# kylc/optik

Hardware: AMD Instinct MI355X
Metric: random-restart IK solves/sec (Panda 7-DoF, 1e-6 tol) (higher is better)
Workload: dtype f64

## Files before the change

include/optik_hip.h:

```cpp
#ifndef OPTIK_HIP_H
#define OPTIK_HIP_H

#include <stdint.h>

#ifdef __cplusplus
extern "C" {
#endif

#define OPTIK_HIP_MAX_DOF 16

enum {
    OPTIK_HIP_OK = 0,
    OPTIK_HIP_EINVAL = -1,
    OPTIK_HIP_EUNSUPPORTED = -2,
    OPTIK_HIP_ENODEVICE = -3,
    OPTIK_HIP_ENOMEM = -4
};

enum { OPTIK_JOINT_FIXED = 0, OPTIK_JOINT_REVOLUTE = 1, OPTIK_JOINT_PRISMATIC = 2 };

enum {
    OPTIK_RES_FAILURE = -1,
    OPTIK_RES_ROUNDOFF_LIMITED = -4,
    OPTIK_RES_FORCED_STOP = -5,
// ... 46 lines not shown
int optik_hip_diff_ik_batch(const optik_hip_chain *chain, const double *ee_offset7, const double *d_q,
                            const double *d_V, int64_t ld_V, const double *d_vmax, int64_t ld_vmax,
                            int64_t B, double *d_alpha, double *d_v, int32_t *d_status, void *stream);

int optik_hip_manip_batch(const optik_hip_chain *chain, const double *ee_offset7, const double *d_q, int64_t B,
                          double *d_w, double *d_c, void *stream);

#define OPTIK_HIP_MAX_COLLISION_SPHERES 256
#define OPTIK_HIP_MAX_COLLISION_PAIRS 4096
#define OPTIK_HIP_MAX_WORLD_OBSTACLES 65536
int optik_hip_chain_set_collision_model(optik_hip_chain *chain, const int32_t *frames, const double *centers3,
                                        const double *radii, int32_t S, const int32_t *pairs2, int32_t P,
                                        double margin);
int optik_hip_chain_set_world(optik_hip_chain *chain, const double *spheres4, int32_t Ms, const double *boxes10,
                              int32_t Mb);
int optik_hip_link_frames_batch(const optik_hip_chain *chain, const double *ee_offset7, const double *d_q, int64_t B,
                                double *d_frames, void *stream);
int optik_hip_collision_batch(const optik_hip_chain *chain, const double *ee_offset7, const double *d_q, int64_t B,
                              double *d_clearance, uint8_t *d_free, void *stream);

int optik_hip_seed_batch(const optik_hip_chain *chain, uint64_t first, int64_t count, double *d_q,
                         void *stream);

#define OPTIK_HIP_IK_EARLY_EXIT 1u
#define OPTIK_HIP_IK_FIND_ANY 2u
#define OPTIK_HIP_IK_RESTART_MAJOR 4u
typedef struct optik_hip_ik_outputs {
    double *d_x;
    double *d_f;
    int32_t *d_status;
    int32_t *d_evals;
    double *d_win_x;
    double *d_win_f;
    uint64_t *d_win_idx;
    double *d_win_key;
} optik_hip_ik_outputs;

int optik_hip_ik_batch(optik_hip_chain *chain, const optik_solver_config *cfg,
                       const double *d_targets, const double *d_x0, int32_t T,
                       const double *ee_offset7, uint64_t restart_begin, uint64_t restart_end,
                       uint32_t flags, double deadline_s, const optik_hip_ik_outputs *out,
                       void *stream);

#define OPTIK_HIP_MAX_SOLUTIONS 256
typedef struct optik_hip_ik_solutions_outputs {
    int32_t *d_count;
// ... 50 lines not shown
```

optik_amd/_native.py:

```python
from __future__ import annotations

import ctypes as C
import os

_HERE = os.path.dirname(os.path.abspath(__file__))
LIB_PATH = os.path.join(_HERE, "csrc", "liboptik_amd.so")
if os.environ.get("OPTIK_AMD_LIB"):
    LIB_PATH = os.path.abspath(os.environ["OPTIK_AMD_LIB"])

MAX_DOF = 8
IK_EARLY_EXIT = 1
IK_FIND_ANY = 2
IK_RESTART_MAJOR = 4
UINT64_MAX = 0xFFFFFFFFFFFFFFFF

RES_FAILURE, RES_ROUNDOFF, RES_FORCED_STOP, RES_ITER_CAP = -1, -4, -5, -100
RES_STOPVAL, RES_FTOL, RES_XTOL = 2, 3, 4
RANGE_SINGLE_INCLUSIVE, RANGE_NEW_INCLUSIVE = 0, 1


class OptikHipError(RuntimeError):
    pass


# ... 63 lines not shown
def lib():
    global _lib
    if _lib is not None:
        return _lib
    if not os.path.exists(LIB_PATH):
        raise OptikHipError(
            f"{LIB_PATH} is missing: build it with `python -c 'import __graft_entry__ as g; "
            "g.build()'` (hipcc --offload-arch=gfx950).  optik_amd has no CPU fallback.")
    L = C.CDLL(LIB_PATH, mode=C.RTLD_GLOBAL)
    vp, dp, ip = C.c_void_p, C.POINTER(C.c_double), C.POINTER(C.c_int32)
    L.optik_hip_device_count.restype = C.c_int
    L.optik_hip_set_option.argtypes = [C.c_char_p, C.c_longlong]
    L.optik_hip_get_option.argtypes = [C.c_char_p]
    L.optik_hip_get_option.restype = C.c_longlong
    L.optik_hip_last_error.restype = C.c_char_p
    L.optik_hip_chain_create.argtypes = [dp, dp, ip, C.c_int32, dp, dp, C.c_int32, C.POINTER(vp)]
    L.optik_hip_chain_destroy.argtypes = [vp]
    L.optik_hip_chain_num_positions.argtypes = [vp]
    L.optik_hip_chain_set_range_rule.argtypes = [vp, C.c_int32]
    L.optik_hip_chain_range_rule.argtypes = [vp]
    L.optik_hip_eval_batch.argtypes = [vp, C.POINTER(SolverConfigC), dp, dp, vp, C.c_int64, vp, vp, vp]
    L.optik_hip_fk_batch.argtypes = [vp, dp, vp, C.c_int64, vp, vp, vp]
    L.optik_hip_seed_batch.argtypes = [vp, C.c_uint64, C.c_int64, vp, vp]
    L.optik_hip_manip_batch.argtypes = [vp, dp, vp, C.c_int64, vp, vp, vp]
    ip = C.POINTER(C.c_int32)
    L.optik_hip_chain_set_collision_model.argtypes = [vp, ip, dp, dp, C.c_int32, ip, C.c_int32, C.c_double]
    L.optik_hip_chain_set_world.argtypes = [vp, dp, C.c_int32, dp, C.c_int32]
    L.optik_hip_link_frames_batch.argtypes = [vp, dp, vp, C.c_int64, vp, vp]
    L.optik_hip_collision_batch.argtypes = [vp, dp, vp, C.c_int64, vp, vp, vp]
    L.optik_hip_diff_ik_batch.argtypes = [vp, dp, vp, vp, C.c_int64, vp, C.c_int64, C.c_int64, vp, vp, vp, vp]
    L.optik_hip_ik_batch.argtypes = [vp, C.POINTER(SolverConfigC), vp, vp, C.c_int32, dp,
                                     C.c_uint64, C.c_uint64, C.c_uint32, C.c_double,
                                     C.POINTER(IkOutputs), vp]
    L.optik_hip_ik_solutions.argtypes = [vp, C.POINTER(SolverConfigC), vp, vp, C.c_int32, dp, C.c_uint64,
                                         C.c_uint64, C.c_double, C.c_int32, C.c_double,
                                         C.POINTER(IkSolutionsOutputs), vp]
    L.optik_hip_ik_path.argtypes = [vp, C.POINTER(SolverConfigC), vp, vp, C.c_int32, C.c_int32, dp, C.c_uint64,
                                    C.c_uint64, C.c_uint32, C.c_double, C.c_double, C.POINTER(IkPathOutputs), vp]
    L.optik_hip_ik_host.argtypes = [vp, C.POINTER(SolverConfigC), dp, dp, C.c_int32, dp,
                                    C.c_uint64, C.c_uint64, C.c_uint32, C.c_double, dp, dp,
                                    C.POINTER(C.c_uint64), dp]
    L.optik_hip_probe.argtypes = [C.c_int32, dp, dp, C.c_int64, dp]
    L.optik_hip_probe_math.argtypes = [C.c_int32, dp, C.c_int64, dp]
    L.optik_hip_set_timing.argtypes = [vp, C.c_int32]
    L.optik_hip_last_launch.argtypes = [vp, C.POINTER(LaunchInfo)]
    L.optik_hip_timing_mean.argtypes = [vp, C.POINTER(C.c_double), C.POINTER(C.c_int32)]
# ... 63 lines not shown
```

optik_amd/csrc/ik_batch_ops.hip:

```cpp
#include "diff_ik_lp.hpp"
#include "ik_host.hpp"
#include "ik_jacobian.hpp"

using namespace optik;
using namespace optik::host;
using namespace optik::hostparams;

namespace {

struct EvalLaunch {
    const ChainDev *chain;
    EvalParams ep;
    double target[7];
    const double *q;
    long long B;
    double *f;
    double *g;
};

template <int N, bool TIP>
__global__ __launch_bounds__(256) void eval_batch_kernel(const EvalLaunch a) {
    __shared__ ChainDev sch;
    stage_chain(sch, a.chain);
    const Pose target = load_pose(a.target);
// ... 140 lines not shown
        const double p[7] = {ee.t.x, ee.t.y, ee.t.z, ee.q.i, ee.q.j, ee.q.k, ee.q.w};
#pragma unroll
        for (int i = 0; i < 7; ++i) a.pose[(size_t)i * a.B + b] = p[i];
    }
}

struct SeedLaunch {
    uint32_t key[8];
    double lb[MAX_DOF];
    double scale[MAX_DOF];
    unsigned long long first;
    long long count;
    double *q;
};

template <int N>
__global__ __launch_bounds__(256) void seed_batch_kernel(const SeedLaunch a) {
    for (long long b = (long long)blockIdx.x * blockDim.x + threadIdx.x; b < a.count;
         b += (long long)gridDim.x * blockDim.x) {
        double q[N];
        restart_seed<N>(a.key, a.lb, a.scale, a.first + (unsigned long long)b, q);
#pragma unroll
        for (int i = 0; i < N; ++i) a.q[(size_t)i * a.count + b] = q[i];
    }
}

__global__ void probe_kernel(int op, const double *a, const double *b, long long count, double *out) {
    for (long long i = (long long)blockIdx.x * blockDim.x + threadIdx.x; i < count;
         i += (long long)gridDim.x * blockDim.x) {
        double r = 0.0, s, c;
        switch (op) {
        case 0: r = a[i] / b[i]; break;
        case 1: r = __builtin_sqrt(a[i]); break;
        case 2: sincos_dev(a[i], s, c); r = s; break;
        case 3: sincos_dev(a[i], s, c); r = c; break;
        default: r = atan2_q1(a[i], b[i]); break;
        }
        out[i] = r;
    }
}

__global__ void probe_math_kernel(int op, const double *poses, long long count, double *out, int stride) {
    for (long long i = (long long)blockIdx.x * blockDim.x + threadIdx.x; i < count;
         i += (long long)gridDim.x * blockDim.x) {
        const Pose X = load_pose(poses + i * 7);
        double *o = out + i * stride;
// ... 4 lines not shown
        if (op == 1) {
            for (int r = 0; r < 3; ++r) for (int c = 0; c < 3; ++c) o[r * 3 + c] = Jr.m[r][c];
        } else if (op == 2) {
            const V3 lin = se3_log_linear(rt, X.t);
            o[0] = lin.x; o[1] = lin.y; o[2] = lin.z; o[3] = w.x; o[4] = w.y; o[5] = w.z;
        } else {
            const M3 Q = se3_q_matrix(rt, X.t, Jr);
            for (int r = 0; r < 3; ++r)
                for (int c = 0; c < 3; ++c) {
                    o[r * 6 + c] = Jr.m[r][c];
                    o[r * 6 + 3 + c] = Q.m[r][c];
                    o[(r + 3) * 6 + c] = 0.0;
                    o[(r + 3) * 6 + 3 + c] = Jr.m[r][c];
                }
        }
    }
}

const char *const kPrismaticJacobianMsg =
    "joint_jacobian: prismatic joints are not implemented (the reference panics: kinematics.rs:185 todo!())";

}

extern "C" {

int optik_hip_eval_batch(const optik_hip_chain *ch, const optik_solver_config *cfg, const double *target7,
                         const double *ee_offset7, const double *d_q, int64_t B, double *d_f, double *d_g,
                         void *stream) {
    if (!ch || !cfg || !target7 || !d_q || !d_f || B < 0) return fail(OPTIK_HIP_EINVAL, "bad argument");
    if (B == 0) return 0;
    if (ch->prismatic)
        return fail(OPTIK_HIP_EUNSUPPORTED,
                    "prismatic joints: only forward kinematics is available (the reference's Jacobian panics, kinematics.rs:185)");
    BIND_DEVICE(ch);
    if (ch->wide) {
        WideBatchLaunch w;
        std::memset(&w, 0, sizeof w);
        w.chain = ch->wdev;
        make_eval_params(cfg->linear_weight, cfg->angular_weight, ee_offset7, w.ep);
        std::memcpy(w.target, target7, sizeof w.target);
        w.q = d_q; w.B = B; w.f = d_f; w.g = d_g;
        HIP_TRY(wide_batch_launch(0, grid_for(ch, B, 256, 8), (hipStream_t)stream, w));
        return 0;
    }
    EvalLaunch a;
    a.chain = ch->dev;
// ... 87 lines not shown
    BIND_DEVICE(ch);
    if (ch->wide) {
        WideBatchLaunch w;
        std::memset(&w, 0, sizeof w);
        w.chain = ch->wdev;
        std::memcpy(w.key, ch->key, sizeof w.key);
        w.first = first; w.B = count; w.q_out = d_q;
        HIP_TRY(wide_batch_launch(2, grid_for(ch, count, 256, 8), (hipStream_t)stream, w));
        return 0;
    }
    SeedLaunch a;
    std::memcpy(a.key, ch->key, sizeof a.key);
    std::memcpy(a.lb, ch->host.lb, sizeof a.lb);
    std::memcpy(a.scale, ch->scale, sizeof a.scale);
    a.first = first; a.count = count; a.q = d_q;
    const int grid = grid_for(ch, count, 256, 8);
#define CALL(NN, TT) hipLaunchKernelGGL((seed_batch_kernel<NN>), dim3(grid), dim3(256), 0, (hipStream_t)stream, a)
    OPTIK_DISPATCH(ch, CALL);
#undef CALL
    HIP_TRY(hipGetLastError());
    return 0;
}

int optik_hip_probe(int32_t op, const double *a, const double *b, int64_t count, double *out) {
    if (!a || !out || count < 0) return fail(OPTIK_HIP_EINVAL, "bad argument");
    if (int rc = ensure_device()) return rc;
    if (count == 0) return 0;
    double *d_a = nullptr, *d_b = nullptr, *d_o = nullptr;
    const size_t bytes = sizeof(double) * (size_t)count;
    HIP_TRY(hipMalloc(&d_a, bytes));
    HIP_TRY(hipMalloc(&d_b, bytes));
    HIP_TRY(hipMalloc(&d_o, bytes));
    HIP_TRY(hipMemcpy(d_a, a, bytes, hipMemcpyHostToDevice));
    HIP_TRY(hipMemcpy(d_b, b ? b : a, bytes, hipMemcpyHostToDevice));
    hipLaunchKernelGGL(probe_kernel, dim3(1024), dim3(256), 0, nullptr, op, d_a, d_b, (long long)count, d_o);
    HIP_TRY(hipGetLastError());
    HIP_TRY(hipMemcpy(out, d_o, bytes, hipMemcpyDeviceToHost));
    hipFree(d_a); hipFree(d_b); hipFree(d_o);
    return 0;
}

int optik_hip_probe_math(int32_t op, const double *poses7, int64_t count, double *out) {
    if (!poses7 || !out || count < 0 || op < 0 || op > 3) return fail(OPTIK_HIP_EINVAL, "bad argument");
    if (int rc = ensure_device()) return rc;
    if (count == 0) return 0;
    const int stride = op == 0 ? 3 : (op == 1 ? 9 : (op == 2 ? 6 : 36));
// ... 15 lines not shown
```

optik_amd/csrc/ik_capi.hip:

```cpp
#include <algorithm>
#include <cstdio>
#include <cstdlib>
#include <vector>

#include "ik_host.hpp"

using namespace optik;
using namespace optik::host;
using namespace optik::hostparams;

namespace optik {
namespace host {

thread_local std::string g_err;

static int solve_kernel_from(const char *e) {
    if (!e) return SK_AUTO;
    if (!std::strcmp(e, "quad")) return SK_QUAD;
    if (!std::strcmp(e, "lane64")) return SK_LANE64;
    if (!std::strcmp(e, "general")) return SK_GENERAL;
    return SK_AUTO;
}
Options &opt() {
    static Options o = [] {
        Options v;
        v.solve_kernel = solve_kernel_from(std::getenv("OPTIK_SOLVE_KERNEL"));
        if (const char *e = std::getenv("OPTIK_WIDE_FORM")) v.wide_form = std::strcmp(e, "hbm") == 0 ? 1 : 0;
        if (const char *e = std::getenv("OPTIK_RANDOM_RANGE_RULE"))
            if (std::strcmp(e, "new_inclusive") == 0 || std::strcmp(e, "1") == 0) v.range_rule = OPTIK_HIP_RANGE_NEW_INCLUSIVE;
        return v;
    }();
    return o;
}

}
}

namespace {

int default_range_rule() { return opt().range_rule; }

void set_chain_scales(optik_hip_chain *ch, int rule) {
    ch->range_rule = rule;
    for (int k = 0; k < ch->n; ++k) {
        const double lb = ch->wide ? ch->whost.lb[k] : ch->host.lb[k], ub = ch->wide ? ch->whost.ub[k] : ch->host.ub[k];
        ch->scale[k] = (std::isfinite(lb) && std::isfinite(ub)) ? uniform_scale(lb, ub, rule) : NAN;
        if (ch->wide) ch->whost.scale[k] = ch->scale[k];
    }
}

}

// ... 91 lines not shown
    hipDeviceGetAttribute(&ch->wall_clock_khz, hipDeviceAttributeWallClockRate, dev);
    *out = ch;
    return 0;
}

void optik_hip_chain_destroy(optik_hip_chain *ch) {
    if (!ch) return;
    optik::DeviceScope dev_scope(ch->device_id);
    if (ch->claim_pending) (void)hipStreamSynchronize(nullptr);
    if (ch->dev) hipFree(ch->dev);
    if (ch->wdev) hipFree(ch->wdev);
    if (ch->wide_ws) hipFree(ch->wide_ws);
    if (ch->tile_recs) hipFree(ch->tile_recs);
    if (ch->first_success) hipFree(ch->first_success);
    if (ch->sol_pick) hipFree(ch->sol_pick);
    if (ch->path_carry) hipFree(ch->path_carry);
    if (ch->coll_dev) hipFree(ch->coll_dev);
    if (ch->world_dev) hipFree(ch->world_dev);
    if (ch->tmp_x) hipFree(ch->tmp_x);
    if (ch->tmp_f) hipFree(ch->tmp_f);
    if (ch->tmp_key) hipFree(ch->tmp_key);
    if (ch->queue) hipFree(ch->queue);
    if (ch->hw_dev) hipFree(ch->hw_dev);
    if (ch->hw_pin) hipHostFree(ch->hw_pin);
    if (ch->hw_claim) hipHostFree(ch->hw_claim);
    if (ch->claim_done) hipEventDestroy(ch->claim_done);
    for (int i = 0; i < optik_hip_chain::EV_POOL; ++i) {
        if (ch->ev0[i]) hipEventDestroy(ch->ev0[i]);
        if (ch->ev1[i]) hipEventDestroy(ch->ev1[i]);
    }
    delete ch;
}

int32_t optik_hip_chain_num_positions(const optik_hip_chain *ch) { return ch ? ch->n : 0; }

int optik_hip_chain_set_range_rule(optik_hip_chain *ch, int32_t rule) {
    if (!ch || (rule != OPTIK_HIP_RANGE_SINGLE_INCLUSIVE && rule != OPTIK_HIP_RANGE_NEW_INCLUSIVE))
        return fail(OPTIK_HIP_EINVAL, "bad argument");
    std::lock_guard<std::mutex> lock(ch->mu);
    set_chain_scales(ch, rule);
    if (ch->wide) {
        BIND_DEVICE(ch);
        HIP_TRY(hipMemcpy(ch->wdev, &ch->whost, sizeof(WideChainDev), hipMemcpyHostToDevice));
    }
    return 0;
}

int32_t optik_hip_chain_range_rule(const optik_hip_chain *ch) { return ch ? ch->range_rule : -1; }

}

struct SolvedLaunch {
    double *px, *pf, *pk;
    uint64_t R;
    uint64_t tiles_per_target;
    size_t cols;
    size_t fs_clean_after;
    bool early;
};

static int solve_locked(optik_hip_chain *ch, const optik_solver_config *cfg, const double *d_targets,
                        const double *d_x0, int32_t T, const double *ee_offset7, uint64_t restart_begin,
                        uint64_t restart_end, uint32_t flags, double deadline_s, const optik_hip_ik_outputs *out,
// ... 204 lines not shown
    if (early && (flags & OPTIK_HIP_IK_RESTART_MAJOR) && resident > (long long)T * inflight) {
        const long long floor_res = std::max(2 * cap, (long long)T * 32);
        resident = std::max((long long)T * inflight, std::min(resident, floor_res));
    }
    long long lanes = (resident + cap - 1) / cap;
    if (lanes < 1) lanes = 1;
    if (lanes > per_wave_max) lanes = per_wave_max;
    bool wide_lds = false;
    if (widek) {
        wide_lds = opt().wide_form != 1;
        if (wide_lds) lanes = 1;
    }
    a.wq.lanes = (int)lanes;
    if (claim_request && quadk && !lanek && a.wq.find_any && T == 1 && ch->hw_claim) {
        a.wq.claim = ch->hw_claim;
        a.wq.claim_seq = ++ch->claim_seq;
        if (claim_armed) *claim_armed = true;
        if (stream == nullptr) ch->claim_pending = true;
    }
    long long grid_ll = (resident + lanes - 1) / lanes;
    if (grid_ll > cap) grid_ll = cap;
    const int grid = (int)grid_ll;

    const int ev_slot = ch->ev_count % optik_hip_chain::EV_POOL;
    if (ch->timing) {
        if (!ch->ev0[ev_slot]) { HIP_TRY(hipEventCreate(&ch->ev0[ev_slot])); HIP_TRY(hipEventCreate(&ch->ev1[ev_slot])); }
        HIP_TRY(hipEventRecord(ch->ev0[ev_slot], stream));
    }
    int lds = 0;
    if (widek) {
        const bool lds_form = wide_lds;
        if (!lds_form && (size_t)grid > ch->wide_ws_waves) {
            if (ch->wide_ws) HIP_TRY(hipFree(ch->wide_ws));
            ch->wide_ws = nullptr; ch->wide_ws_waves = 0;
            HIP_TRY(hipMalloc(&ch->wide_ws, sizeof(double) * wide_ws_doubles_per_wave() * (size_t)grid));
            ch->wide_ws_waves = (size_t)grid;
        }
        WideSolveLaunch w;
        std::memset(&w, 0, sizeof w);
        w.chain = ch->wdev;
        w.ep = a.ep; w.sp = a.sp; w.wq = a.wq;
        std::memcpy(w.key, ch->key, sizeof w.key);
        w.deadline_ticks = a.deadline_ticks;
        w.ws = ch->wide_ws;
        lds = lds_form ? wide_lds_bytes() : (int)sizeof(WideChainDev);
        HIP_TRY(wide_solve_launch(grid, stream, w, lds_form, opt().wide_form != 2));
// ... 120 lines not shown
        s.x = out->d_x ? out->d_x + w * (size_t)n : nullptr;
        s.f = out->d_f ? out->d_f + w : nullptr;
        s.idx = out->d_idx ? (unsigned long long *)out->d_idx + w : nullptr;
        s.key = out->d_key ? out->d_key + w : nullptr;
        s.step = out->d_step ? out->d_step + w : nullptr;
        s.reset_queue = ch->queue;
        s.reset_fs = sl.early ? ch->first_success : nullptr;
        HIP_TRY(path_select_launch(s, P, stream));
        ch->queue_clean = true;
        ch->fs_clean = sl.fs_clean_after;
        ch->clean_stream = stream;
    }
    return 0;
}

static long long *option_slot(const char *name, int **islot) {
    Options &o = opt();
    *islot = nullptr;
    if (!name) return nullptr;
    if (!std::strcmp(name, "solve_kernel")) { *islot = &o.solve_kernel; return nullptr; }
    if (!std::strcmp(name, "wide_form")) { *islot = &o.wide_form; return nullptr; }
    if (!std::strcmp(name, "range_rule")) { *islot = &o.range_rule; return nullptr; }
    if (!std::strcmp(name, "stop_x_legacy")) { *islot = &o.stop_x_legacy; return nullptr; }
    return nullptr;
}
int optik_hip_set_option(const char *name, long long value) {
    int *is = nullptr;
    long long *ls = option_slot(name, &is);
    if (ls) { *ls = value; return 0; }
    if (is) { *is = (int)value; return 0; }
    return fail(OPTIK_HIP_EINVAL, "unknown option");
}
long long optik_hip_get_option(const char *name) {
    int *is = nullptr;
    long long *ls = option_slot(name, &is);
    return ls ? *ls : (is ? (long long)*is : -1);
}

int optik_hip_ik_host(optik_hip_chain *ch, const optik_solver_config *cfg, const double *targets,
                      const double *x0, int32_t T, const double *ee_offset7, uint64_t restart_begin,
                      uint64_t restart_end, uint32_t flags, double deadline_s, double *win_x, double *win_f,
                      uint64_t *win_idx, double *win_key) {
    if (!ch || !cfg || !targets || !x0 || T < 1) return fail(OPTIK_HIP_EINVAL, "bad argument");
    std::lock_guard<std::mutex> host_lock(ch->host_mu);
    BIND_DEVICE(ch);
    const int n = ch->n;
// ... 132 lines not shown
```

optik_amd/csrc/ik_host.hpp:

```cpp
#pragma once

#include <hip/hip_runtime.h>

#include <cmath>
#include <cstring>
#include <mutex>
#include <string>

#include "../../include/optik_hip.h"
#include "device_scope.hpp"
#include "ik_host_params.hpp"
#include "ik_launch.hpp"
#include "ik_wide_launch.hpp"

namespace optik {
namespace coll {
struct ModelDev;
}
namespace host {

constexpr int WAVE = 64;
constexpr int QUADS_PER_WAVE_HOST = 16;

struct TileRec {
// ... 57 lines not shown
    int n;
    int filter;
    double max_step;
    unsigned long long restart_begin;
    unsigned long long n_restarts;
    size_t ld;
    double *x;
    double *f;
    unsigned long long *idx;
    double *key;
    double *step;
    unsigned long long *reset_queue;
    unsigned long long *reset_fs;
};
hipError_t path_select_launch(const PathSelectLaunch &s, int P, hipStream_t stream);

int manip_key_launch(const optik_hip_chain *ch, int mode, const double *ee_offset7, const double *x, double *key,
                     size_t cols, hipStream_t stream);

int collision_key_launch(const optik_hip_chain *ch, const double *ee_offset7, const double *x, double *key,
                         size_t cols, hipStream_t stream);

enum : int { SK_AUTO = 0, SK_QUAD = 1, SK_LANE64 = 2, SK_GENERAL = 3 };
struct Options {
    int solve_kernel = SK_AUTO;
    int wide_form = 0;
    int range_rule = OPTIK_HIP_RANGE_SINGLE_INCLUSIVE;
    int stop_x_legacy = 0;
};
Options &opt();

extern thread_local std::string g_err;
inline int fail(int code, const std::string &msg) {
    g_err = msg;
    return code;
}

#define HIP_TRY(expr)                                                                   \
    do {                                                                                \
        hipError_t e_ = (expr);                                                         \
        if (e_ != hipSuccess)                                                           \
            return ::optik::host::fail(OPTIK_HIP_ENODEVICE, std::string(#expr) + ": " + hipGetErrorString(e_)); \
    } while (0)

inline int ensure_device() {
    int n = 0;
    hipError_t e = hipGetDeviceCount(&n);
    if (e != hipSuccess || n <= 0)
        return fail(OPTIK_HIP_ENODEVICE, std::string("no HIP device available: ")
                                             + (e == hipSuccess ? "device count is 0" : hipGetErrorString(e)));
    return 0;
// ... 52 lines not shown
    size_t sol_pick_cap = 0;
    double *path_carry = nullptr;
    size_t path_carry_cap = 0;
    int coll_S = 0, coll_P = 0, coll_groups = 0;
    double coll_margin = 0.0;
    optik::coll::ModelDev *coll_dev = nullptr;
    double *world_dev = nullptr;
    size_t world_cap = 0;
    int world_Ms = 0, world_Mb = 0;
    bool queue_clean = false;
    size_t fs_clean = 0;
    hipStream_t clean_stream = nullptr;
    double *tmp_x = nullptr, *tmp_f = nullptr, *tmp_key = nullptr;
    size_t tmp_cols = 0;
    unsigned long long *queue = nullptr;
    unsigned long long *prof = nullptr;
    double *hw_dev = nullptr, *hw_pin = nullptr;
    size_t hw_cap = 0;
    unsigned long long *hw_claim = nullptr;
    hipEvent_t claim_done = nullptr;
    unsigned long long claim_seq = 0;
    bool claim_pending = false;
    unsigned hw_flip = 0;
    int timing = 0;
    static constexpr int EV_POOL = 256;
    hipEvent_t ev0[EV_POOL] = {}, ev1[EV_POOL] = {};
    int ev_count = 0;
    optik_hip_launch_info last{};
    int num_cus = 0;
    int wall_clock_khz = 0;
};

namespace optik {
namespace host {

inline int grid_for(const optik_hip_chain *ch, long long work, int block, int per_cu) {
    long long blocks = (work + block - 1) / block;
    const long long cap = (long long)(ch->num_cus > 0 ? ch->num_cus : 256) * per_cu;
    if (blocks > cap) blocks = cap;
    if (blocks < 1) blocks = 1;
    return (int)blocks;
}

}
}
```

optik_amd/csrc/ik_lane64.hpp:

```cpp
#pragma once

#include "ik_lane.hpp"
#include "ik_solve.hpp"
#include "ik_nnls_quad.hpp"

namespace optik {

template <int N>
struct Lane64Geom {
    static constexpr int NG = N * (N + 1) / 2;
    static constexpr int REC = NG + 2 * N;
    OPTIK_DEV static constexpr int g(int i, int j) { return i * N - (i * (i - 1)) / 2 + (j - i); }
    OPTIK_DEV static constexpr int hlo(int i) { return NG + i; }
    OPTIK_DEV static constexpr int hhi(int i) { return NG + N + i; }
    static constexpr int META = NnlsQuadGeom<N>::XS + 2 * N;
    static_assert(NnlsQuadGeom<N>::XS + 2 * N + 3 <= NnlsQuadGeom<N>::STRIDE, "three spare doubles per block");
};

}
#include "ik_nnls_first.hpp"
namespace optik {

#ifndef OPTIK_LANE_FIRST_PASS_MIN
#define OPTIK_LANE_FIRST_PASS_MIN 16
// ... 7 lines not shown

template <int N>
constexpr int lane64_block_lds() { return nnls_quad_wave_lds<N>(); }
template <int N>
constexpr int lane64_rec_lds() { return Lane64Geom<N>::REC * 64; }

#ifndef OPTIK_LANE_CLASSES
#define OPTIK_LANE_CLASSES 8
#endif
constexpr int LANE64_CLASSES = OPTIK_LANE_CLASSES;
#ifndef OPTIK_LANE_PIPE
#define OPTIK_LANE_PIPE 1
#endif
#ifndef LANE64_MAX_RUNNING
#define LANE64_MAX_RUNNING 14
#endif
#ifndef OPTIK_LANE_RESERVE
#define OPTIK_LANE_RESERVE 8
#endif
#ifndef OPTIK_LANE_KEEP_TARGET
#define OPTIK_LANE_KEEP_TARGET 1
#endif
#ifndef OPTIK_LANE_REFILL
#define OPTIK_LANE_REFILL 4
#endif

template <int N, class Expand, class ReadBack>
struct Lane64Pipe {
    static constexpr bool on = true;
    static constexpr bool warm_start = true;
    static constexpr int MAX_RUNNING = LANE64_MAX_RUNNING;
    int n_prob, next, hold;
    int qi, ql, lane, rank;
    bool has, got;
    double *bk;
    int *lor, *where;
    Expand *expand_fn;
    ReadBack *read_fn;
    OPTIK_DEV bool more() const { return next < n_prob; }
    template <bool WARM>
    OPTIK_DEV bool event(bool idle, int mode, double rn, int passes, double *wst, int &wj) {
        wj = 0;
        const bool fin = idle && hold >= 0;
        if (wave_any(fin)) {
            if (fin && ql == 0) {
                bk[Lane64Geom<N>::META] = (double)mode;
                bk[Lane64Geom<N>::META + 1] = rn;
                bk[Lane64Geom<N>::META + 2] = (double)passes;
// ... 8 lines not shown
            if (fin) hold = -1;
        }
        const bool free_q = idle && hold < 0;
        const unsigned long long fm = __ballot(free_q);
        const int mine = (int)__popcll(fm & ((1ull << (lane & ~3)) - 1ull)) / QUAD;
        const int pr = next + mine;
        const bool live = free_q && pr < n_prob;
        next += (int)__popcll(fm) / QUAD;
        next = next < n_prob ? next : n_prob;
        if (wave_any(live)) {
            const int p = lor[live ? pr : 0];
            (*expand_fn)(std::integral_constant<bool, WARM>{}, live, p, wst, wj);
            if (live) hold = pr;
        }
        return live;
    }
};

template <int N, bool TIP>
OPTIK_DEV void lane64_wave(const ChainDev &ch, const EvalParams &ep, const SolveParams &sp, const uint32_t (&key)[8],
                           const double (&scale)[MAX_DOF], const WorkQueue &wq,
                           double *nnls_lds ,
                           double *rec_lds , int *lor_lds ,
                           int *where_lds ) {
    typedef Lane64Geom<N> G;
    constexpr int NL = N * (N + 1) / 2;
    constexpr int NS = (N > 4) ? 2 : 1;
    constexpr int CS = NnlsQuadGeom<N>::CS;
    static_assert(N <= 7, "the throughput form of chains with at most seven joints");
    const double alfmin = 0.1;
    const int lane = (int)(threadIdx.x & 63u);
    double x[N], x0[N], g[N], s[N], l[NL];
    double xbest[N], xprev[N];
    double f = 0.0, f0 = 0.0, t0 = 0.0, h3 = 0.0, alpha = 1.0;
    double minf = __builtin_huge_val(), fprev = __builtin_huge_val();
    int ireset = 0, line = 0, nevals = 0;
    int pred = 1;
    bool first = true;
    bool again = false;
    Pose target;
    unsigned long long item = 0, index = 0;
    unsigned tslot = OPTIK_LANE_KEEP_TARGET ? ~0u : 0u;
    bool active = false, want = lane < wq.lanes;
#if OPTIK_LANE_RESERVE > 0
    unsigned long long rbase = 0, rend = 0;
    unsigned long long pend = 0;
    bool r_pending = false;
    bool dry = false;
#endif
#pragma unroll
    for (int i = 0; i < N; ++i) { x[i] = 0.0; x0[i] = 0.0; g[i] = 0.0; s[i] = 0.0; xbest[i] = 0.0; xprev[i] = 0.0; }
#pragma unroll
    for (int i = 0; i < NL; ++i) l[i] = 0.0;
    target.t = V3{0, 0, 0};
    target.q = Q4{0, 0, 0, 1};

#ifdef OPTIK_PROFILE
    unsigned long long lp_[8] = {0, 0, 0, 0, 0, 0, 0, 0};
    unsigned long long lt_ = __builtin_readcyclecounter();
#define LANE_PROF(slot) do { const unsigned long long n_ = __builtin_readcyclecounter(); lp_[slot] += n_ - lt_; lt_ = n_; } while (0)
#else
#define LANE_PROF(slot)
#endif
    for (;;) {
        const unsigned n_want = (unsigned)__popcll(__ballot(want));
        if (n_want >= (unsigned)(wq.lanes < OPTIK_LANE_REFILL ? wq.lanes : OPTIK_LANE_REFILL) || (n_want > 0 && !wave_any(active))) {
#if OPTIK_LANE_RESERVE > 0
            unsigned long long it;
            {
                if (r_pending) { rbase = __shfl(pend, 0); rend = rbase + OPTIK_LANE_RESERVE; r_pending = false; }
                const unsigned long long wm = __ballot(want);
                const unsigned rank = (unsigned)__popcll(wm & ((1ull << lane) - 1ull));
                const unsigned long long have = rend - rbase;
                const unsigned long long take = n_want < have ? n_want : have;
                it = rbase + rank;
                rbase += take;
                if (wave_any(want && rank >= take)) {
                    const unsigned long long it2 = fetch_items(wq.next_item, want && rank >= take);
                    if (rank >= take) it = it2;
                }
                dry = dry || wave_any(want && it >= wq.total_items);
            }
#else
            const unsigned long long it = fetch_items(wq.next_item, want);
#endif
            if (want) {
                want = false;
                if (it < wq.total_items) {
                    unsigned long long r;
#if OPTIK_LANE_KEEP_TARGET
                    const unsigned tprev = tslot;
#endif
                    if (wq.restart_major) { r = it / wq.n_targets; tslot = (unsigned)(it - r * wq.n_targets); }
                    else { tslot = (unsigned)(it / wq.n_restarts); r = it - (unsigned long long)tslot * wq.n_restarts; }
                    item = (unsigned long long)tslot * wq.n_restarts + r;
                    index = wq.restart_begin + r;
#if OPTIK_LANE_KEEP_TARGET
                    if (tslot != tprev) target = load_pose(wq.targets + (size_t)tslot * 7);
#else
                    target = load_pose(wq.targets + (size_t)tslot * 7);
#endif
                    restart_seed<N>(key, ch.lb, scale, index, x);
                    if (index == 0) {
                        const double *x0p = wq.x0 + (size_t)tslot * N;
#pragma unroll
                        for (int i = 0; i < N; ++i) x[i] = x0p[i];
                    }
#pragma unroll
                    for (int i = 0; i < N; ++i) { xbest[i] = x[i]; xprev[i] = x[i]; x0[i] = x[i]; s[i] = 0.0; g[i] = 0.0; }
                    f = 0.0; f0 = 0.0; t0 = 0.0; h3 = 0.0; alpha = 1.0;
                    minf = __builtin_huge_val(); fprev = __builtin_huge_val();
                    ireset = 0; line = 0; nevals = 0; pred = 1;
                    first = true;
                    again = false;
                    active = true;
                }
            }
        }
#if OPTIK_LANE_RESERVE > 0
        if (!r_pending && rbase == rend && !dry) {
            if (lane == 0) pend = atomicAdd(wq.next_item, (unsigned long long)OPTIK_LANE_RESERVE);
            r_pending = true;
        }
#endif
        if (!wave_any(active)) break;
        LANE_PROF(0);

        int32_t ret = 0;
        if (active) {
            bool stop = false;
            if (wq.first_success) {
                const unsigned long long fs = __hip_atomic_load(wq.first_success + tslot, __ATOMIC_RELAXED,
                                                                __HIP_MEMORY_SCOPE_AGENT);
                stop = wq.find_any ? (fs != ~0ull) : (fs < index);
            }
            if (wq.deadline && (unsigned long long)wall_clock64() > wq.deadline) stop = true;
            if (stop) ret = RES_FORCED_STOP;
        }
        const bool stepping = active && ret == 0;
        const bool do_eval = stepping && !again;
        double gn[N];
        double fn = 0.0;
        OPTIK_SCHED_FENCE_LANE64();
        if (do_eval) fn = eval_fg<N, TIP>(ch, ep, target, x, gn);
        OPTIK_SCHED_FENCE_LANE64();
        LANE_PROF(1);

        bool need_dir = stepping && again, reset = stepping && again;
        again = false;
        if (do_eval) {
            f = fn;
            ++nevals;
            if (f < minf) {
                minf = f;
#pragma unroll
                for (int i = 0; i < N; ++i) xbest[i] = x[i];
            }
            if (minf < sp.stopval) {
                ret = RES_STOPVAL_REACHED;
            } else if (nevals >= MAX_EVALS_CAP) {
                ret = RES_ITER_CAP;
            } else if (first) {
                first = false;
#pragma unroll
                for (int i = 0; i < N; ++i) g[i] = gn[i];
                need_dir = true;
                reset = true;
            } else {
// ... 315 lines not shown
            double k = __builtin_huge_val();
            if (success) {
                if (wq.quality) {
                    const double *x0p = wq.x0 + (size_t)tslot * N;
                    double acc = 0.0;
#pragma unroll
                    for (int i = 0; i < N; ++i) { const double d = xbest[i] - x0p[i]; acc += d * d; }
                    k = __builtin_sqrt(acc);
                } else {
                    k = (double)index;
                    if (wq.first_success) atomicMin(wq.first_success + tslot, index);
                }
            }
            if (wq.out_key) wq.out_key[item] = k;
            active = false;
            want = true;
            again = false;
        }
#ifdef OPTIK_PROFILE
        LANE_PROF(3);
        lp_[7] += 1;
#endif
    }
#ifdef OPTIK_PROFILE
    if (wq.prof && (threadIdx.x & 63u) == 0)
        for (int i_ = 0; i_ < 8; ++i_) atomicAdd(wq.prof + i_, lp_[i_]);
#endif
#undef LANE_PROF
}

}
```

optik_amd/csrc/ik_lane_kernel.hip:

```cpp
#include <hip/hip_runtime.h>

#include "ik_launch.hpp"
#include "ik_lane64.hpp"

namespace optik {

template <int N, bool TIP>
__global__ __launch_bounds__(64, 1) void ik_lane_kernel(const SolveLaunch a) {
    __shared__ ChainDev sch;
    __shared__ __attribute__((aligned(16))) double nnls_lds[lane64_block_lds<N>()];
    __shared__ __attribute__((aligned(16))) double rec_lds[lane64_rec_lds<N>()];
    __shared__ int lor_lds[64], where_lds[64];
    __shared__ __attribute__((aligned(8))) uint32_t launch_lds[(sizeof(SolveLaunch) + 3) / 4];
    {
        const uint32_t *src = reinterpret_cast<const uint32_t *>(&a);
        for (unsigned i = threadIdx.x; i < sizeof(SolveLaunch) / 4; i += 64) launch_lds[i] = src[i];
    }
    if (threadIdx.x < 16) nnls_lds[lane64_block_lds<N>() - 16 + threadIdx.x] = 0.0;
    lor_lds[threadIdx.x & 63u] = 0;
    where_lds[threadIdx.x & 63u] = 0;
    stage_chain(sch, a.chain);
    SolveLaunch &L = *reinterpret_cast<SolveLaunch *>(launch_lds);
    if (threadIdx.x == 0) L.wq.deadline = L.deadline_ticks ? wall_clock64() + L.deadline_ticks : 0ull;
    __syncthreads();
    lane64_wave<N, TIP>(sch, L.ep, L.sp, L.key, L.scale, L.wq, nnls_lds, rec_lds, lor_lds, where_lds);
}

int lane_solve_waves_per_cu() { return 4; }

hipError_t lane_solve_launch(int n, bool tip, int grid, hipStream_t stream, const SolveLaunch &a, int *lds_bytes) {
    if (lds_bytes)
        *lds_bytes = (int)(sizeof(ChainDev) + sizeof(SolveLaunch) + 128 * sizeof(int)
                           + sizeof(double) * (lane64_block_lds<7>() + lane64_rec_lds<7>()));
#define CALL_LANE(NN)                                                                                  \
    case NN:                                                                                           \
        if (tip) hipLaunchKernelGGL((ik_lane_kernel<NN, true>), dim3(grid), dim3(64), 0, stream, a);   \
        else hipLaunchKernelGGL((ik_lane_kernel<NN, false>), dim3(grid), dim3(64), 0, stream, a);      \
        break;
    switch (n) {
#ifdef OPTIK_LANE_ONLY_N
        CALL_LANE(OPTIK_LANE_ONLY_N)
#else
        CALL_LANE(1) CALL_LANE(2) CALL_LANE(3) CALL_LANE(4) CALL_LANE(5) CALL_LANE(6) CALL_LANE(7)
#endif
    default: return hipErrorInvalidValue;
    }
#undef CALL_LANE
    return hipGetLastError();
}

}

#ifdef OPTIK_PROFILE
extern "C" int optik_hip_lane_nnls_hist(unsigned long long *out66) {
    if (hipDeviceSynchronize() != hipSuccess) return -1;
    if (hipMemcpyFromSymbol(out66, HIP_SYMBOL(optik::g_quad_nnls_hist), 66 * sizeof(unsigned long long)) != hipSuccess) return -1;
// ... 13 lines not shown
```

optik_amd/csrc/ik_solve.hpp:

```cpp
#pragma once

#include "ik_slsqp.hpp"

namespace optik {

enum : int32_t {
    RES_FAILURE = -1,
    RES_ROUNDOFF_LIMITED = -4,
    RES_FORCED_STOP = -5,
    RES_ITER_CAP = -100,
    RES_STOPVAL_REACHED = 2,
    RES_FTOL_REACHED = 3,
    RES_XTOL_REACHED = 4,
};

constexpr int MAX_EVALS_CAP = 100000;
constexpr unsigned REFILL_BATCH = 8;

#ifdef OPTIK_PROFILE
#define OPTIK_PROF_DECL unsigned long long prof_[8] = {0, 0, 0, 0, 0, 0, 0, 0}; unsigned long long prof_t_ = 0
#define OPTIK_PROF_BEGIN() prof_t_ = __builtin_readcyclecounter()
#define OPTIK_PROF_END(slot) prof_[slot] += __builtin_readcyclecounter() - prof_t_
#define OPTIK_PROF_COUNT(slot, n) prof_[slot] += (n)
#define OPTIK_PROF_SUB_BEGIN() const unsigned long long prof_s_ = __builtin_readcyclecounter()
// ... 84 lines not shown

struct WorkQueue {
    unsigned long long *next_item;
    unsigned long long total_items;
    unsigned long long n_restarts;
    unsigned long long restart_begin;
    const double *targets;
    const double *x0;
    unsigned long long *first_success;
    int find_any;
    int restart_major;
    unsigned long long n_targets;
    unsigned long long deadline;
    int quality;
    int lanes;
    double *out_x;
    double *out_f;
    double *out_key;
    int32_t *out_status;
    int32_t *out_evals;
    unsigned long long *prof;
    unsigned long long *claim;
    unsigned long long claim_seq;
};

OPTIK_DEV unsigned long long fetch_items(unsigned long long *counter, bool want) {
    const unsigned long long mask = __ballot(want);
    const unsigned n = (unsigned)__popcll(mask);
    unsigned long long base = 0;
    if (n) {
        const int leader = __ffsll((long long)mask) - 1;
        const int lane = (int)(threadIdx.x & 63u);
        if (lane == leader) base = atomicAdd(counter, (unsigned long long)n);
        base = __shfl(base, leader, 64);
    }
    const unsigned rank = (unsigned)__popcll(mask & ((1ull << (threadIdx.x & 63u)) - 1ull));
    return base + rank;
}

}
```

optik_amd/device.py:

```python
from __future__ import annotations

import ctypes as C

import numpy as np
import torch

from . import _native as nat


def _stream_ptr():
    return C.c_void_p(torch.cuda.current_stream().cuda_stream)


def _ptr(t):
    return C.c_void_p(t.data_ptr()) if t is not None else C.c_void_p(None)


def _dp(a):
    return a.ctypes.data_as(C.POINTER(C.c_double))


class HipChain:

    def __init__(self, types, origins, axes, lb, ub, device="cuda:0"):
# ... 108 lines not shown
        return ee

    def link_frames_batch(self, q, ee_offset7=None):
        B = self._check_q(q)
        ee = self._ee7(ee_offset7)
        frames = torch.empty((B, self.n + 2, 7), dtype=torch.float64, device=q.device)
        nat.check(nat.lib().optik_hip_link_frames_batch(self._h, _dp(ee) if ee is not None else None, _ptr(q), B,
                                                        _ptr(frames), _stream_ptr()))
        return frames

    def collision_batch(self, q, ee_offset7=None):
        B = self._check_q(q)
        ee = self._ee7(ee_offset7)
        clearance = torch.empty(B, dtype=torch.float64, device=q.device)
        free = torch.empty(B, dtype=torch.uint8, device=q.device)
        nat.check(nat.lib().optik_hip_collision_batch(self._h, _dp(ee) if ee is not None else None, _ptr(q), B,
                                                      _ptr(clearance), _ptr(free), _stream_ptr()))
        return clearance, free.bool()

    def seed_batch(self, first, count):
        q = torch.empty((self.n, count), dtype=torch.float64, device=self.device)
        nat.check(nat.lib().optik_hip_seed_batch(self._h, int(first), int(count), _ptr(q), _stream_ptr()))
        return q

    def alloc_ik_buffers(self, T, R, per_restart=True):
        dev = self.device
        bufs = dict(
            win_x=torch.empty((T, self.n), dtype=torch.float64, device=dev),
            win_f=torch.empty(T, dtype=torch.float64, device=dev),
            win_idx=torch.empty(T, dtype=torch.int64, device=dev),
            win_key=torch.empty(T, dtype=torch.float64, device=dev))
        if per_restart:
            bufs.update(
                x=torch.empty((self.n, T * R), dtype=torch.float64, device=dev),
                f=torch.empty(T * R, dtype=torch.float64, device=dev),
                status=torch.empty(T * R, dtype=torch.int32, device=dev),
                evals=torch.empty(T * R, dtype=torch.int32, device=dev))
        return bufs

    def ik_batch(self, cfg, targets, x0, restart_begin, restart_end, flags=0, deadline_s=0.0,
                 ee_offset7=None, bufs=None, per_restart=True):
        assert targets.is_cuda and targets.dtype == torch.float64 and targets.is_contiguous()
        assert x0.is_cuda and x0.dtype == torch.float64 and x0.is_contiguous()
        T = targets.shape[0]
        assert targets.shape == (T, 7) and x0.shape == (T, self.n)
        R = int(restart_end - restart_begin)
# ... 124 lines not shown
```

Measured before the change: 35.63 million.

## Serve random-restart seeds from a cached device table with LDS prefetch

Adds a per-chain device table of precomputed restart seeds, filled lazily by a new kernel and padded to 8-double rows. The lane64 solver reads seeds from this table instead of running the restart_seed generator. For reserved work items it prefetches rows into LDS with global_load_lds and waits on them after the eval phase. The lane refill threshold also drops from 4 to 2. This trades on-device RNG cost for memory traffic, extra LDS, a first-call build with a stream synchronize, and a table of up to 2^20 rows by default.

```diff
diff --git a/include/optik_hip.h b/include/optik_hip.h
--- a/include/optik_hip.h
+++ b/include/optik_hip.h
@@ -92,6 +92,10 @@
 int optik_hip_seed_batch(const optik_hip_chain *chain, uint64_t first, int64_t count, double *d_q,
                          void *stream);
 
+uint64_t optik_hip_seed_table_plan(uint64_t restart_end, long long cap, uint64_t have);
+int optik_hip_seed_table_read(optik_hip_chain *chain, uint64_t first, int64_t count, double *d_rows, int64_t *copied,
+                              void *stream);
+
 #define OPTIK_HIP_IK_EARLY_EXIT 1u
 #define OPTIK_HIP_IK_FIND_ANY 2u
 #define OPTIK_HIP_IK_RESTART_MAJOR 4u
diff --git a/optik_amd/_native.py b/optik_amd/_native.py
--- a/optik_amd/_native.py
+++ b/optik_amd/_native.py
@@ -109,6 +109,9 @@
     L.optik_hip_eval_batch.argtypes = [vp, C.POINTER(SolverConfigC), dp, dp, vp, C.c_int64, vp, vp, vp]
     L.optik_hip_fk_batch.argtypes = [vp, dp, vp, C.c_int64, vp, vp, vp]
     L.optik_hip_seed_batch.argtypes = [vp, C.c_uint64, C.c_int64, vp, vp]
+    L.optik_hip_seed_table_plan.argtypes = [C.c_uint64, C.c_longlong, C.c_uint64]
+    L.optik_hip_seed_table_plan.restype = C.c_uint64
+    L.optik_hip_seed_table_read.argtypes = [vp, C.c_uint64, C.c_int64, vp, C.POINTER(C.c_int64), vp]
     L.optik_hip_manip_batch.argtypes = [vp, dp, vp, C.c_int64, vp, vp, vp]
     ip = C.POINTER(C.c_int32)
     L.optik_hip_chain_set_collision_model.argtypes = [vp, ip, dp, dp, C.c_int32, ip, C.c_int32, C.c_double]
diff --git a/optik_amd/csrc/ik_batch_ops.hip b/optik_amd/csrc/ik_batch_ops.hip
--- a/optik_amd/csrc/ik_batch_ops.hip
+++ b/optik_amd/csrc/ik_batch_ops.hip
@@ -186,6 +186,20 @@
         restart_seed<N>(a.key, a.lb, a.scale, a.first + (unsigned long long)b, q);
 #pragma unroll
         for (int i = 0; i < N; ++i) a.q[(size_t)i * a.count + b] = q[i];
+    }
+}
+
+template <int N>
+__global__ __launch_bounds__(256) void seed_table_kernel(const SeedLaunch a) {
+    for (long long b = (long long)blockIdx.x * blockDim.x + threadIdx.x; b < a.count;
+         b += (long long)gridDim.x * blockDim.x) {
+        double q[N];
+        restart_seed<N>(a.key, a.lb, a.scale, a.first + (unsigned long long)b, q);
+        double *row = a.q + (a.first + (unsigned long long)b) * SEED_ROW;
+#pragma unroll
+        for (int i = 0; i < N; ++i) row[i] = q[i];
+#pragma unroll
+        for (int i = N; i < SEED_ROW; ++i) row[i] = 0.0;
     }
 }
 
@@ -236,6 +250,46 @@
 
 }
 
+namespace optik {
+namespace host {
+
+int seed_table_ensure(optik_hip_chain *ch, unsigned long long restart_end, hipStream_t stream, const double **table,
+                      unsigned long long *rows) {
+    *table = nullptr;
+    *rows = 0;
+    if (ch->wide || ch->prismatic || ch->n > SEED_ROW) return 0;
+    for (int k = 0; k < ch->n; ++k)
+        if (std::isnan(ch->scale[k])) return 0;
+    const unsigned long long want = seed_table_rows_for(restart_end, opt().seed_table_rows, ch->seed_rows);
+    if (want > ch->seed_rows) {
+        if (want > ch->seed_cap) {
+            if (ch->seed_table) HIP_TRY(hipFree(ch->seed_table));
+            ch->seed_table = nullptr; ch->seed_cap = 0; ch->seed_rows = 0;
+            HIP_TRY(hipMalloc(&ch->seed_table, sizeof(double) * SEED_ROW * (size_t)want));
+            ch->seed_cap = want;
+        }
+        SeedLaunch a;
+        std::memcpy(a.key, ch->key, sizeof a.key);
+        std::memcpy(a.lb, ch->host.lb, sizeof a.lb);
+        std::memcpy(a.scale, ch->scale, sizeof a.scale);
+        a.first = ch->seed_rows; a.count = (long long)(want - ch->seed_rows); a.q = ch->seed_table;
+        const int grid = grid_for(ch, a.count, 256, 8);
+#define CALL(NN, TT) hipLaunchKernelGGL((seed_table_kernel<NN>), dim3(grid), dim3(256), 0, stream, a)
+        OPTIK_DISPATCH(ch, CALL);
+#undef CALL
+        HIP_TRY(hipGetLastError());
+        HIP_TRY(hipStreamSynchronize(stream));
+        ch->seed_rows = want;
+    }
+    const unsigned long long cap = opt().seed_table_rows <= 0 ? 0ull : (unsigned long long)opt().seed_table_rows;
+    *rows = ch->seed_rows < cap ? ch->seed_rows : cap;
+    *table = *rows ? ch->seed_table : nullptr;
+    return 0;
+}
+
+}
+}
+
 extern "C" {
 
 int optik_hip_eval_batch(const optik_hip_chain *ch, const optik_solver_config *cfg, const double *target7,
@@ -369,6 +423,28 @@
     return 0;
 }
 
+uint64_t optik_hip_seed_table_plan(uint64_t restart_end, long long cap, uint64_t have) {
+    return seed_table_rows_for(restart_end, cap, have);
+}
+
+int optik_hip_seed_table_read(optik_hip_chain *ch, uint64_t first, int64_t count, double *d_rows, int64_t *copied,
+                              void *stream) {
+    if (!ch || !d_rows || !copied || count < 0) return fail(OPTIK_HIP_EINVAL, "bad argument");
+    *copied = 0;
+    if (ch->wide || ch->prismatic) return fail(OPTIK_HIP_EUNSUPPORTED, "the seed table serves revolute chains of at most 8 joints");
+    std::lock_guard<std::mutex> lock(ch->mu);
+    BIND_DEVICE(ch);
+    const double *table = nullptr;
+    unsigned long long rows = 0;
+    if (int rc = seed_table_ensure(ch, first + (uint64_t)count, (hipStream_t)stream, &table, &rows)) return rc;
+    if (first >= rows || count == 0) return 0;
+    const uint64_t n = std::min<uint64_t>((uint64_t)count, rows - first);
+    HIP_TRY(hipMemcpyAsync(d_rows, table + first * SEED_ROW, sizeof(double) * SEED_ROW * n, hipMemcpyDeviceToDevice,
+                           (hipStream_t)stream));
+    *copied = (int64_t)n;
+    return 0;
+}
+
 int optik_hip_probe(int32_t op, const double *a, const double *b, int64_t count, double *out) {
     if (!a || !out || count < 0) return fail(OPTIK_HIP_EINVAL, "bad argument");
     if (int rc = ensure_device()) return rc;
diff --git a/optik_amd/csrc/ik_capi.hip b/optik_amd/csrc/ik_capi.hip
--- a/optik_amd/csrc/ik_capi.hip
+++ b/optik_amd/csrc/ik_capi.hip
@@ -28,6 +28,7 @@
         if (const char *e = std::getenv("OPTIK_WIDE_FORM")) v.wide_form = std::strcmp(e, "hbm") == 0 ? 1 : 0;
         if (const char *e = std::getenv("OPTIK_RANDOM_RANGE_RULE"))
             if (std::strcmp(e, "new_inclusive") == 0 || std::strcmp(e, "1") == 0) v.range_rule = OPTIK_HIP_RANGE_NEW_INCLUSIVE;
+        if (const char *e = std::getenv("OPTIK_SEED_TABLE_ROWS")) v.seed_table_rows = std::atoll(e);
         return v;
     }();
     return o;
@@ -165,6 +166,7 @@
     if (ch->tmp_key) hipFree(ch->tmp_key);
     if (ch->queue) hipFree(ch->queue);
     if (ch->hw_dev) hipFree(ch->hw_dev);
+    if (ch->seed_table) hipFree(ch->seed_table);
     if (ch->hw_pin) hipHostFree(ch->hw_pin);
     if (ch->hw_claim) hipHostFree(ch->hw_claim);
     if (ch->claim_done) hipEventDestroy(ch->claim_done);
@@ -182,6 +184,7 @@
         return fail(OPTIK_HIP_EINVAL, "bad argument");
     std::lock_guard<std::mutex> lock(ch->mu);
     set_chain_scales(ch, rule);
+    ch->seed_rows = 0;
     if (ch->wide) {
         BIND_DEVICE(ch);
         HIP_TRY(hipMemcpy(ch->wdev, &ch->whost, sizeof(WideChainDev), hipMemcpyHostToDevice));
@@ -432,6 +435,8 @@
     if (grid_ll > cap) grid_ll = cap;
     const int grid = (int)grid_ll;
 
+    if (lanek && !widek)
+        if (int rc = seed_table_ensure(ch, restart_end, stream, &a.wq.seed_table, &a.wq.seed_rows)) return rc;
     const int ev_slot = ch->ev_count % optik_hip_chain::EV_POOL;
     if (ch->timing) {
         if (!ch->ev0[ev_slot]) { HIP_TRY(hipEventCreate(&ch->ev0[ev_slot])); HIP_TRY(hipEventCreate(&ch->ev1[ev_slot])); }
@@ -598,6 +603,7 @@
     if (!std::strcmp(name, "wide_form")) { *islot = &o.wide_form; return nullptr; }
     if (!std::strcmp(name, "range_rule")) { *islot = &o.range_rule; return nullptr; }
     if (!std::strcmp(name, "stop_x_legacy")) { *islot = &o.stop_x_legacy; return nullptr; }
+    if (!std::strcmp(name, "seed_table_rows")) return &o.seed_table_rows;
     return nullptr;
 }
 int optik_hip_set_option(const char *name, long long value) {
diff --git a/optik_amd/csrc/ik_host.hpp b/optik_amd/csrc/ik_host.hpp
--- a/optik_amd/csrc/ik_host.hpp
+++ b/optik_amd/csrc/ik_host.hpp
@@ -103,11 +103,21 @@
                          size_t cols, hipStream_t stream);
 
 enum : int { SK_AUTO = 0, SK_QUAD = 1, SK_LANE64 = 2, SK_GENERAL = 3 };
+constexpr long long SEED_TABLE_DEFAULT_ROWS = 1ll << 20;
+constexpr long long SEED_TABLE_MAX_ROWS = 1ll << 26;
+inline unsigned long long seed_table_rows_for(unsigned long long restart_end, long long cap, unsigned long long have) {
+    const unsigned long long c = cap <= 0 ? 0ull : (unsigned long long)(cap < SEED_TABLE_MAX_ROWS ? cap : SEED_TABLE_MAX_ROWS);
+    unsigned long long want = restart_end < c ? restart_end : c;
+    if (want <= have) return have;
+    want = (want + 4095ull) & ~4095ull;
+    return want < c ? want : c;
+}
 struct Options {
     int solve_kernel = SK_AUTO;
     int wide_form = 0;
     int range_rule = OPTIK_HIP_RANGE_SINGLE_INCLUSIVE;
     int stop_x_legacy = 0;
+    long long seed_table_rows = SEED_TABLE_DEFAULT_ROWS;
 };
 Options &opt();
 
@@ -206,6 +216,9 @@
     unsigned long long claim_seq = 0;
     bool claim_pending = false;
     unsigned hw_flip = 0;
+    double *seed_table = nullptr;
+    unsigned long long seed_rows = 0;
+    unsigned long long seed_cap = 0;
     int timing = 0;
     static constexpr int EV_POOL = 256;
     hipEvent_t ev0[EV_POOL] = {}, ev1[EV_POOL] = {};
@@ -218,6 +231,9 @@
 namespace optik {
 namespace host {
 
+int seed_table_ensure(optik_hip_chain *ch, unsigned long long restart_end, hipStream_t stream, const double **table,
+                      unsigned long long *rows);
+
 inline int grid_for(const optik_hip_chain *ch, long long work, int block, int per_cu) {
     long long blocks = (work + block - 1) / block;
     const long long cap = (long long)(ch->num_cus > 0 ? ch->num_cus : 256) * per_cu;
diff --git a/optik_amd/csrc/ik_lane64.hpp b/optik_amd/csrc/ik_lane64.hpp
--- a/optik_amd/csrc/ik_lane64.hpp
+++ b/optik_amd/csrc/ik_lane64.hpp
@@ -53,8 +53,31 @@
 #define OPTIK_LANE_KEEP_TARGET 1
 #endif
 #ifndef OPTIK_LANE_REFILL
-#define OPTIK_LANE_REFILL 4
-#endif
+#define OPTIK_LANE_REFILL 2
+#endif
+
+#ifndef OPTIK_LANE_SEED_TABLE
+#define OPTIK_LANE_SEED_TABLE 1
+#endif
+
+constexpr int lane64_seed_lds() { return (OPTIK_LANE_RESERVE > 0 ? OPTIK_LANE_RESERVE : 1) * SEED_ROW; }
+static_assert(4 * OPTIK_LANE_RESERVE <= 64, "a row of the seed table moves as four 16-byte pieces, one per lane");
+
+OPTIK_DEV void seed_piece_to_lds(const double *src, double *dst) {
+#ifdef OPTIK_LANE_EMU
+    double *d = dst + 2 * (int)(threadIdx.x & 63u);
+    d[0] = src[0];
+    d[1] = src[1];
+#else
+    __builtin_amdgcn_global_load_lds((const __attribute__((address_space(1))) void *)src,
+                                     (__attribute__((address_space(3))) void *)dst, 16, 0, 0);
+#endif
+}
+OPTIK_DEV void seed_pieces_landed() {
+#ifndef OPTIK_LANE_EMU
+    __builtin_amdgcn_s_waitcnt(0x0f70);
+#endif
+}
 
 template <int N, class Expand, class ReadBack>
 struct Lane64Pipe {
@@ -109,7 +132,8 @@
                            const double (&scale)[MAX_DOF], const WorkQueue &wq,
                            double *nnls_lds ,
                            double *rec_lds , int *lor_lds ,
-                           int *where_lds ) {
+                           int *where_lds ,
+                           double *seed_lds = nullptr ) {
     typedef Lane64Geom<N> G;
     constexpr int NL = N * (N + 1) / 2;
     constexpr int NS = (N > 4) ? 2 : 1;
@@ -154,13 +178,16 @@
         if (n_want >= (unsigned)(wq.lanes < OPTIK_LANE_REFILL ? wq.lanes : OPTIK_LANE_REFILL) || (n_want > 0 && !wave_any(active))) {
 #if OPTIK_LANE_RESERVE > 0
             unsigned long long it;
+            bool parked;
+            unsigned slot;
             {
-                if (r_pending) { rbase = __shfl(pend, 0); rend = rbase + OPTIK_LANE_RESERVE; r_pending = false; }
                 const unsigned long long wm = __ballot(want);
                 const unsigned rank = (unsigned)__popcll(wm & ((1ull << lane) - 1ull));
                 const unsigned long long have = rend - rbase;
                 const unsigned long long take = n_want < have ? n_want : have;
                 it = rbase + rank;
+                parked = rank < take;
+                slot = (unsigned)(OPTIK_LANE_RESERVE - (rend - it));
                 rbase += take;
                 if (wave_any(want && rank >= take)) {
                     const unsigned long long it2 = fetch_items(wq.next_item, want && rank >= take);
@@ -170,6 +197,8 @@
             }
 #else
             const unsigned long long it = fetch_items(wq.next_item, want);
+            const bool parked = false;
+            const unsigned slot = 0;
 #endif
             if (want) {
                 want = false;
@@ -187,7 +216,20 @@
 #else
                     target = load_pose(wq.targets + (size_t)tslot * 7);
 #endif
-                    restart_seed<N>(key, ch.lb, scale, index, x);
+#if OPTIK_LANE_SEED_TABLE
+                    if (index < wq.seed_rows) {
+                        if (parked) {
+                            const double *row = seed_lds + slot * SEED_ROW;
+#pragma unroll
+                            for (int i = 0; i < N; ++i) x[i] = row[i];
+                        } else {
+                            const double *row = (const double *)__builtin_assume_aligned(wq.seed_table + index * SEED_ROW, 64);
+#pragma unroll
+                            for (int i = 0; i < N; ++i) x[i] = row[i];
+                        }
+                    } else
+#endif
+                        restart_seed<N>(key, ch.lb, scale, index, x);
                     if (index == 0) {
                         const double *x0p = wq.x0 + (size_t)tslot * N;
 #pragma unroll
@@ -205,7 +247,26 @@
             }
         }
 #if OPTIK_LANE_RESERVE > 0
-        if (!r_pending && rbase == rend && !dry) {
+        if (rbase == rend && r_pending) {
+            rbase = __shfl(pend, 0);
+            rend = rbase + OPTIK_LANE_RESERVE;
+            r_pending = false;
+            dry = dry || rbase >= wq.total_items;
+#if OPTIK_LANE_SEED_TABLE
+            if (wq.seed_rows) {
+                lds_sync();
+                const unsigned long long pit = rbase + (unsigned)(lane >> 2);
+                if (lane < 4 * OPTIK_LANE_RESERVE && pit < wq.total_items) {
+                    unsigned long long r;
+                    if (wq.restart_major) r = pit / wq.n_targets;
+                    else r = pit % wq.n_restarts;
+                    const unsigned long long pidx = wq.restart_begin + r;
+                    if (pidx < wq.seed_rows) seed_piece_to_lds(wq.seed_table + pidx * SEED_ROW + 2 * (lane & 3), seed_lds);
+                }
+            }
+#endif
+        }
+        if (!r_pending && !dry) {
             if (lane == 0) pend = atomicAdd(wq.next_item, (unsigned long long)OPTIK_LANE_RESERVE);
             r_pending = true;
         }
@@ -231,6 +292,9 @@
         OPTIK_SCHED_FENCE_LANE64();
         if (do_eval) fn = eval_fg<N, TIP>(ch, ep, target, x, gn);
         OPTIK_SCHED_FENCE_LANE64();
+#if OPTIK_LANE_RESERVE > 0 && OPTIK_LANE_SEED_TABLE
+        seed_pieces_landed();
+#endif
         LANE_PROF(1);
 
         bool need_dir = stepping && again, reset = stepping && again;
@@ -592,6 +656,9 @@
         lp_[7] += 1;
 #endif
     }
+#if OPTIK_LANE_RESERVE > 0 && OPTIK_LANE_SEED_TABLE
+    seed_pieces_landed();
+#endif
 #ifdef OPTIK_PROFILE
     if (wq.prof && (threadIdx.x & 63u) == 0)
         for (int i_ = 0; i_ < 8; ++i_) atomicAdd(wq.prof + i_, lp_[i_]);
diff --git a/optik_amd/csrc/ik_lane_kernel.hip b/optik_amd/csrc/ik_lane_kernel.hip
--- a/optik_amd/csrc/ik_lane_kernel.hip
+++ b/optik_amd/csrc/ik_lane_kernel.hip
@@ -11,6 +11,7 @@
     __shared__ __attribute__((aligned(16))) double nnls_lds[lane64_block_lds<N>()];
     __shared__ __attribute__((aligned(16))) double rec_lds[lane64_rec_lds<N>()];
     __shared__ int lor_lds[64], where_lds[64];
+    __shared__ __attribute__((aligned(64))) double seed_lds[lane64_seed_lds()];
     __shared__ __attribute__((aligned(8))) uint32_t launch_lds[(sizeof(SolveLaunch) + 3) / 4];
     {
         const uint32_t *src = reinterpret_cast<const uint32_t *>(&a);
@@ -23,7 +24,7 @@
     SolveLaunch &L = *reinterpret_cast<SolveLaunch *>(launch_lds);
     if (threadIdx.x == 0) L.wq.deadline = L.deadline_ticks ? wall_clock64() + L.deadline_ticks : 0ull;
     __syncthreads();
-    lane64_wave<N, TIP>(sch, L.ep, L.sp, L.key, L.scale, L.wq, nnls_lds, rec_lds, lor_lds, where_lds);
+    lane64_wave<N, TIP>(sch, L.ep, L.sp, L.key, L.scale, L.wq, nnls_lds, rec_lds, lor_lds, where_lds, seed_lds);
 }
 
 int lane_solve_waves_per_cu() { return 4; }
@@ -31,7 +32,7 @@
 hipError_t lane_solve_launch(int n, bool tip, int grid, hipStream_t stream, const SolveLaunch &a, int *lds_bytes) {
     if (lds_bytes)
         *lds_bytes = (int)(sizeof(ChainDev) + sizeof(SolveLaunch) + 128 * sizeof(int)
-                           + sizeof(double) * (lane64_block_lds<7>() + lane64_rec_lds<7>()));
+                           + sizeof(double) * (lane64_block_lds<7>() + lane64_rec_lds<7>() + lane64_seed_lds()));
 #define CALL_LANE(NN)                                                                                  \
     case NN:                                                                                           \
         if (tip) hipLaunchKernelGGL((ik_lane_kernel<NN, true>), dim3(grid), dim3(64), 0, stream, a);   \
diff --git a/optik_amd/csrc/ik_solve.hpp b/optik_amd/csrc/ik_solve.hpp
--- a/optik_amd/csrc/ik_solve.hpp
+++ b/optik_amd/csrc/ik_solve.hpp
@@ -130,7 +130,11 @@
     unsigned long long *prof;
     unsigned long long *claim;
     unsigned long long claim_seq;
+    const double *seed_table;
+    unsigned long long seed_rows;
 };
+
+constexpr int SEED_ROW = 8;
 
 OPTIK_DEV unsigned long long fetch_items(unsigned long long *counter, bool want) {
     const unsigned long long mask = __ballot(want);
diff --git a/optik_amd/device.py b/optik_amd/device.py
--- a/optik_amd/device.py
+++ b/optik_amd/device.py
@@ -154,6 +154,13 @@
         q = torch.empty((self.n, count), dtype=torch.float64, device=self.device)
         nat.check(nat.lib().optik_hip_seed_batch(self._h, int(first), int(count), _ptr(q), _stream_ptr()))
         return q
+
+    def seed_table_rows(self, first, count):
+        rows = torch.empty((max(int(count), 1), 8), dtype=torch.float64, device=self.device)
+        copied = C.c_int64(0)
+        nat.check(nat.lib().optik_hip_seed_table_read(self._h, int(first), int(count), _ptr(rows), C.byref(copied),
+                                                      _stream_ptr()))
+        return rows[:copied.value]
 
     def alloc_ik_buffers(self, T, R, per_restart=True):
         dev = self.device
```

Result: no change. 35.93 million (median of 6 runs) (+0.8%).
